# scverse/scanpy

Hardware: AMD Instinct MI355X
Metric: cells/sec through pca+neighbors+leiden, 1M x 2k CSR (higher is better)
Workload: dtype bf16x3

## Files before the change

### include/scanpy_amd.h

```cpp
#ifndef SCANPY_AMD_H
#define SCANPY_AMD_H

#include <stddef.h>
#include <stdint.h>

#ifdef __cplusplus
extern "C" {
#endif

typedef struct ihipStream_t* scamd_stream_t;

#define SCAMD_OK 0
#define SCAMD_EINVAL (-1)
#define SCAMD_EWORKSPACE (-2)
#define SCAMD_EHIP (-3)
#define SCAMD_EUNSUPPORTED (-4)
#define SCAMD_ECAPACITY (-5)
#define SCAMD_EINTERNAL (-6)

#define SCAMD_ABI_VERSION 1

int scamd_abi_version(void);
const char* scamd_last_error(void);
int scamd_device_count(void);

size_t scamd_knn_workspace_bytes(int64_t n, int d, int64_t n_query, int k);
int scamd_knn_l2_f32(const float* x, int64_t n, int d, int64_t ld_x,
                     int64_t q_begin, int64_t n_query, int k,
                     int32_t* out_idx, double* out_dist,
                     double cert_scale, int64_t* n_fallback_host,
                     void* workspace, size_t workspace_bytes, scamd_stream_t stream);
int scamd_knn_l2_ivf_f32(const float* x, int64_t n, int d, int64_t ld_x,
                         int64_t q_begin, int64_t n_query, int k, int nprobe,
                         int32_t* out_idx, double* out_dist, int64_t* n_fallback_host,
                         void* workspace, size_t workspace_bytes, scamd_stream_t stream);
float scamd_knn_last_select_ms(void);
double scamd_knn_last_select_pairs(void);
double scamd_knn_last_select_prepass_pairs(void);
int scamd_knn_last_select_engine(void);
int scamd_knn_last_second_tier_queries(void);
int scamd_knn_last_nprobe(void);
int scamd_knn_last_coarse(void);
void scamd_knn_cert_factors(int engine, double* cert_k, double* cert_k2, double* key_slack);
size_t scamd_knn_debug_b3_scores_workspace_bytes(int64_t n);
int scamd_knn_debug_b3_scores_f32(const float* x, int64_t n, int d, int64_t ld_x, int64_t q0, int nq, int64_t c0, int nc,
                                  float* out_scores, float* out_mu, float* out_cmax, void* workspace,
                                  size_t workspace_bytes, scamd_stream_t stream);
int scamd_knn_debug_cell_tables_sizes(int64_t n, int d, int64_t n_query, int k, int nprobe, int* n_cells, int64_t* n_img_max);
int scamd_knn_debug_cell_tables(int64_t n, int d, int64_t n_query, int k, int nprobe, const void* workspace,
                                size_t workspace_bytes, int32_t* out_labels, int32_t* out_row_cell, int32_t* out_cell_map,
                                float* out_cent, float* out_radius, int32_t* out_tile0, int32_t* out_ntiles, int32_t* out_order,
                                float* out_lb2, int32_t* out_perm, int64_t* n_img_rows_host, scamd_stream_t stream);
int scamd_knn_debug_sweep_tables(int64_t n, int d, int64_t n_query, int k, int nprobe, const void* workspace,
                                 size_t workspace_bytes, float* out_reach, int32_t* out_list_len, int32_t* out_sweep_order,
                                 float* out_sweep_lb2, scamd_stream_t stream);

size_t scamd_fuzzy_workspace_bytes(int64_t n, int k);
int scamd_fuzzy_simplicial_set_f32(const int32_t* knn_idx, const float* knn_dist, int64_t n, int k,
                                   int64_t* out_indptr, int32_t* out_indices, float* out_data,
                                   int64_t cap, float* out_sigma, float* out_rho, int64_t* nnz_host,
                                   void* workspace, size_t workspace_bytes, scamd_stream_t stream);
int scamd_fuzzy_weights_f32(const int32_t* knn_idx, const float* knn_dist, int64_t n_local, int k, int64_t row_begin,
                            int64_t n_total, const double* sum_all_dev, float* w, float* out_sigma, float* out_rho,
                            int32_t* out_count, scamd_stream_t stream);
size_t scamd_fuzzy_merge_workspace_bytes(int64_t n_local, int64_t cap);
int scamd_fuzzy_merge_rows_f32(const int32_t* knn_idx, const float* w, int64_t n_local, int k, const int64_t* in_indptr,
                               const int32_t* in_src, const float* in_w, int64_t* out_indptr, int32_t* out_indices,
                               float* out_data, int64_t cap, int64_t* nnz_host, void* workspace, size_t workspace_bytes,
                               scamd_stream_t stream);
int scamd_gauss_connectivities_f32(const int32_t* knn_idx, const float* knn_dist, int64_t n, int k, int64_t* out_indptr,
                                   int32_t* out_indices, float* out_data, int64_t cap, int64_t* nnz_host,
                                   void* workspace, size_t workspace_bytes, scamd_stream_t stream);
int scamd_jaccard_connectivities_f32(const int32_t* knn_idx, int64_t n, int k, int64_t* out_indptr,
                                     int32_t* out_indices, float* out_data, int64_t cap, int64_t* nnz_host,
                                     void* workspace, size_t workspace_bytes, scamd_stream_t stream);


int scamd_csr_row_stats_f32(const int64_t* indptr, const float* data, int64_t n_rows,
                            double* row_sum, double* row_sumsq, scamd_stream_t stream);
size_t scamd_csr_transpose_workspace_bytes(int64_t n, int64_t g, int64_t nnz);
int scamd_csr_transpose_f32(const int64_t* indptr, const int32_t* indices, const float* data,
                            int64_t n, int64_t g, int64_t nnz,
                            int64_t* t_indptr, int32_t* t_indices, float* t_data,
                            void* workspace, size_t workspace_bytes, scamd_stream_t stream);
int scamd_spmm_csr_f32(const int64_t* indptr, const int32_t* indices, const float* data,
// ... 246 lines not shown
```

### scanpy_amd/_lib.py

```python
from __future__ import annotations

import ctypes as C
from functools import lru_cache
from pathlib import Path

LIB_PATH = Path(__file__).resolve().parent / "_lib" / "libscanpy_amd.so"

_i64, _i32, _f64, _sz, _vp, _u64 = C.c_int64, C.c_int, C.c_double, C.c_size_t, C.c_void_p, C.c_uint64

SIGNATURES = {
    "scamd_abi_version": (_i32, []),
    "scamd_last_error": (C.c_char_p, []),
    "scamd_device_count": (_i32, []),
    "scamd_knn_workspace_bytes": (_sz, [_i64, _i32, _i64, _i32]),
    "scamd_knn_l2_f32": (_i32, [_vp, _i64, _i32, _i64, _i64, _i64, _i32, _vp, _vp, _f64, C.POINTER(_i64), _vp, _sz, _vp]),
    "scamd_knn_l2_ivf_f32": (_i32, [_vp, _i64, _i32, _i64, _i64, _i64, _i32, _i32, _vp, _vp, C.POINTER(_i64), _vp, _sz, _vp]),
    "scamd_knn_last_select_ms": (C.c_float, []),
    "scamd_knn_last_select_pairs": (_f64, []),
    "scamd_knn_last_select_prepass_pairs": (_f64, []),
    "scamd_knn_last_select_engine": (_i32, []),
    "scamd_knn_last_second_tier_queries": (_i32, []),
    "scamd_knn_last_nprobe": (_i32, []),
    "scamd_knn_last_coarse": (_i32, []),
    "scamd_knn_cert_factors": (None, [_i32, C.POINTER(_f64), C.POINTER(_f64), C.POINTER(_f64)]),
    "scamd_knn_debug_b3_scores_workspace_bytes": (_sz, [_i64]),
    "scamd_knn_debug_b3_scores_f32": (_i32, [_vp, _i64, _i32, _i64, _i64, _i32, _i64, _i32, _vp, _vp, _vp, _vp, _sz, _vp]),
    "scamd_knn_debug_cell_tables_sizes": (_i32, [_i64, _i32, _i64, _i32, _i32, C.POINTER(_i32), C.POINTER(_i64)]),
    "scamd_knn_debug_cell_tables": (_i32, [_i64, _i32, _i64, _i32, _i32, _vp, _sz, _vp, _vp, _vp, _vp, _vp, _vp, _vp, _vp, _vp, _vp,
                                           C.POINTER(_i64), _vp]),
    "scamd_knn_debug_sweep_tables": (_i32, [_i64, _i32, _i64, _i32, _i32, _vp, _sz, _vp, _vp, _vp, _vp, _vp]),
    "scamd_fuzzy_workspace_bytes": (_sz, [_i64, _i32]),
    "scamd_fuzzy_simplicial_set_f32": (_i32, [_vp, _vp, _i64, _i32, _vp, _vp, _vp, _i64, _vp, _vp, C.POINTER(_i64), _vp, _sz, _vp]),
    "scamd_fuzzy_weights_f32": (_i32, [_vp, _vp, _i64, _i32, _i64, _i64, _vp, _vp, _vp, _vp, _vp, _vp]),
    "scamd_fuzzy_merge_workspace_bytes": (_sz, [_i64, _i64]),
    "scamd_fuzzy_merge_rows_f32": (_i32, [_vp, _vp, _i64, _i32, _vp, _vp, _vp, _vp, _vp, _vp, _i64, C.POINTER(_i64), _vp, _sz, _vp]),
    "scamd_gauss_connectivities_f32": (_i32, [_vp, _vp, _i64, _i32, _vp, _vp, _vp, _i64, C.POINTER(_i64), _vp, _sz, _vp]),
    "scamd_jaccard_connectivities_f32": (_i32, [_vp, _i64, _i32, _vp, _vp, _vp, _i64, C.POINTER(_i64), _vp, _sz, _vp]),
    "scamd_csr_row_stats_f32": (_i32, [_vp, _vp, _i64, _vp, _vp, _vp]),
    "scamd_csr_transpose_workspace_bytes": (_sz, [_i64, _i64, _i64]),
    "scamd_csr_transpose_f32": (_i32, [_vp, _vp, _vp, _i64, _i64, _i64, _vp, _vp, _vp, _vp, _sz, _vp]),
    "scamd_spmm_csr_f32": (_i32, [_vp, _vp, _vp, _i64, _i64, _vp, _i32, _vp, _vp, _vp]),
    "scamd_spmm_f64acc_workspace_bytes": (_sz, [_i64, _i64, _i32]),
    "scamd_spmm_csr_f32_f64acc": (_i32, [_vp, _vp, _vp, _i64, _i64, _vp, _i32, _vp, _vp, _vp, _vp, _sz, _vp]),
    "scamd_csr_gram_workspace_bytes": (_sz, [_i64, _i64]),
    "scamd_csr_gram_f32": (_i32, [_vp, _vp, _vp, _i64, _i64, _i64, _i32, _vp, _i64, _vp, C.POINTER(C.c_float), _vp, _sz, _vp]),
    "scamd_eigh_topk_workspace_bytes": (_sz, [_i64, _i32]),
    "scamd_eigh_topk_f64": (_i32, [_vp, _i64, _i64, _i32, _u64, _f64, _vp, _vp, _vp, _vp, _sz, _vp]),
    "scamd_dense_debug_f64": (_i32, [_i32, _vp, _vp, _i32, _i32, _i32, _vp, _vp, C.POINTER(_i32), _vp]),
    "scamd_pca_csr_workspace_bytes": (_sz, [_i64, _i64, _i32]),
    "scamd_pca_csr_f32": (_i32, [_vp, _vp, _vp, _i64, _i64, _i64, _i32, _i32, _u64, _f64, _vp, _vp, _vp, _vp, _vp, _vp, _vp, _sz, _vp]),
    "scamd_pca_solve_gram_workspace_bytes": (_sz, [_i64, _i32]),
    "scamd_pca_solve_gram_f64": (_i32, [_vp, _i64, _vp, _i64, _i64, _i32, _i32, _i32, _u64, _f64, _vp, _vp, _vp, _vp, _vp, _vp, _vp, _vp, _vp, _sz, _vp]),
    "scamd_spectral_embedding_workspace_bytes": (_sz, [_i64, _i64, _i32]),
    "scamd_spectral_embedding_f32": (_i32, [_vp, _vp, _vp, _i64, _i64, _i32, _u64, _f64, _i32, _i32, _vp, C.POINTER(_f64), _vp, _sz, _vp]),
    "scamd_transitions_sym_workspace_bytes": (_sz, [_i64, _i64]),
    "scamd_transitions_sym_f32": (_i32, [_vp, _vp, _vp, _i64, _i64, _i32, _vp, _vp, _vp, _sz, _vp]),
    "scamd_diffmap_workspace_bytes": (_sz, [_i64, _i64, _i32]),
    "scamd_diffmap_f32": (_i32, [_vp, _vp, _vp, _i64, _i64, _i32, _u64, _f64, _i32, _i32, _vp, _vp, C.POINTER(_f64), _vp, _sz, _vp]),
    "scamd_dpt_pseudotime_workspace_bytes": (_sz, [_i64]),
    "scamd_dpt_pseudotime_f32": (_i32, [_vp, _vp, _i64, _i32, _i64, _i64, _vp, _i32, _vp, _vp, _sz, _vp]),
    "scamd_colsum_workspace_bytes": (_sz, [_i32]),
    "scamd_colsum_f32_f64": (_i32, [_vp, _i64, _i32, _vp, _vp, _sz, _vp]),
# ... 129 lines not shown
```

### scanpy_amd/csrc/knn.hip

```cpp
#include "common.h"

#include <algorithm>
#include <cmath>
#include <cstdlib>
#include <memory>
#include <type_traits>
#include <vector>

struct KnnLast {
  float select_ms = -1.f;
  double select_pairs = -1.0, select_prepass_pairs = -1.0;
  int select_engine = -1, second_tier = 0;
  int coarse = 0;
  int nprobe = 0;
};
static thread_local KnnLast g_last;

namespace scamd {

using f32x16 = __attribute__((ext_vector_type(16))) float;
using f32x4 = __attribute__((ext_vector_type(4))) float;
using i32x4 = __attribute__((ext_vector_type(4))) int;
typedef __attribute__((__vector_size__(8 * sizeof(__bf16)))) __bf16 bf16x8;

// ... 1915 lines not shown
    const int64_t i = i0 + (int64_t)t * 1024;
    if (cell[t] < 0) continue;
    const int c = cell[t];
    const int pos = row_off[c] + l_row[c] + rk[t];
    perm[pos] = (int)i;
    if (qk[t] >= 0) {
      qpos[slot_off[c] + l_slot[c] + qk[t]] = pos;
      if (qrow) qrow[i - q0] = pos;
    }
  }
}

__global__ void ivf_t2_count_kernel(const int* __restrict__ flag_list, int n_flag, int64_t q0, const int* __restrict__ labels,
                                    const int* __restrict__ cell_map, int* __restrict__ cnt, int* __restrict__ cell_out,
                                    int* __restrict__ pos_out) {
  const int j = blockIdx.x * blockDim.x + threadIdx.x;
  if (j >= n_flag) return;
  const int c = cell_map[labels[q0 + flag_list[j]]];
  cell_out[j] = c;
  pos_out[j] = atomicAdd(&cnt[c], 1);
}
__global__ void ivf_t2_fill_kernel(const int* __restrict__ flag_list, int n_flag, const int* __restrict__ cell_in,
                                   const int* __restrict__ pos_in, const int* __restrict__ slot_off,
                                   const int* __restrict__ qrow, int* __restrict__ qpos) {
  const int j = blockIdx.x * blockDim.x + threadIdx.x;
  if (j >= n_flag) return;
  qpos[slot_off[cell_in[j]] + pos_in[j]] = qrow[flag_list[j]];
}
__global__ void knn_iota_kernel(int* __restrict__ a, int n) {
  const int i = blockIdx.x * blockDim.x + threadIdx.x;
  if (i < n) a[i] = i;
}

__global__ void ivf_pack_image_kernel(const float* __restrict__ x, const float* __restrict__ mu, int d, int64_t ld,
                                      int H, int HP, int DPL,
                                      int64_t n_img, const int* __restrict__ perm, const int* __restrict__ labels,
                                      const int* __restrict__ cell_map, const float* __restrict__ cent,
                                      float* __restrict__ xp, unsigned int* __restrict__ cmax_bits,
                                      unsigned int* __restrict__ radius_bits, int b3) {
  const int lane = threadIdx.x & 63, sub = lane & 15;
  const int64_t grp = ((int64_t)blockIdx.x * blockDim.x + threadIdx.x) >> 4;
  const int64_t ngrp = ((int64_t)gridDim.x * blockDim.x) >> 4;
  float wmax = 0.f;
  const int64_t rpg = (n_img + ngrp - 1) / ngrp;
  const int64_t r_lo = grp * rpg, r_hi = r_lo + rpg < n_img ? r_lo + rpg : n_img;
  int run_cell = -1;
  unsigned int run_rb = 0u;
  auto flush_radius = [&]() {
    if (sub == 0 && run_cell >= 0 && run_rb > 0u) atomicMax(&radius_bits[run_cell], run_rb);
  };
  int src_next = r_lo < r_hi ? perm[r_lo] : -1;
  for (int64_t r = r_lo; r < r_hi; ++r) {
    const int src = src_next;
    src_next = r + 1 < r_hi ? perm[r + 1] : -1;
    double s = 0.0;
    float dc2 = 0.f;
    int cell = 0;
    if (src >= 0) {
      cell = cell_map[labels[src]];
      for (int c = sub; c < d; c += 16) {
        const float v = x[(int64_t)src * ld + c];
        const float vc = __fsub_rn(v, mu[c]);
        s += (double)vc * (double)vc;
        const float df = v - cent[cell * d + c];
        dc2 = fmaf(df, df, dc2);
      }
    }
#pragma unroll
    for (int o = 8; o > 0; o >>= 1) {
      s += __shfl_xor(s, o);
      dc2 += __shfl_xor(dc2, o);
    }
    const float nf = (src >= 0) ? (float)s : INFINITY;
    pack_image_row(xp, r, sub, 16, b3, H, HP, DPL, d, src < 0, nf,
                   [&](int dim) { return src >= 0 ? __fsub_rn(x[(int64_t)src * ld + dim], mu[dim]) : 0.f; });
    if (src >= 0) {
      wmax = fmaxf(wmax, nf);
      const unsigned int rb = __float_as_uint(sqrtf(dc2) * 1.0001f + 1e-6f);
      if (cell != run_cell) {
        flush_radius();
        run_cell = cell;
        run_rb = 0u;
      }
      run_rb = max(run_rb, rb);
    }
  }
  flush_radius();
#pragma unroll
  for (int o = 32; o > 0; o >>= 1) wmax = fmaxf(wmax, __shfl_xor(wmax, o));
  if (lane == 0 && wmax > 0.f && __float_as_uint(wmax) > __hip_atomic_load(cmax_bits, __ATOMIC_RELAXED, __HIP_MEMORY_SCOPE_AGENT))
    atomicMax(cmax_bits, __float_as_uint(wmax));
}


struct KnnPlan {
  int H, TC, NW, KP;
  bool reg;
  bool b3;
  bool thr_margin_env;
  int thr_rank;
  int row_dwords;
  int64_t n_pad, nq_pad;
  bool ivf;
  int nprobe;
  int n_cells;
  int64_t n_img_max, n_slot_max;
};

static bool knn_plan(int64_t n, int d, int64_t n_query, int k, KnnPlan* p, int nprobe = 0) {
  p->nprobe = 0;
  if (d <= 16) p->H = 8;
  else if (d <= 32) p->H = 16;
  else if (d <= 50) p->H = 25;
  else if (d <= 64) p->H = 32;
  else if (d <= 128) p->H = 64;
  else if (d <= 256) p->H = 128;
  else return false;
  p->TC = (p->H == 128) ? 32 : ((p->H == 64) ? 64 : 128);
  if (k <= 24) { p->KP = 32; p->NW = 8; }
  else if (k <= 56) { p->KP = 64; p->NW = 4; }
// ... 89 lines not shown
    b->block_perm = ws.take<int>(block_perm_capacity(p));
    b->qorder = ws.take<int>((size_t)p.n_slot_max);
    b->reach = ws.take<float>((size_t)p.n_cells * p.n_cells);
    b->list_len = ws.take<int>((size_t)p.n_cells);
    b->reach_chunks = ws.take<int>((size_t)p.n_cells);
    b->sweep_order = ws.take<int>((size_t)p.n_cells * p.n_cells);
    b->sweep_lb2 = ws.take<float>((size_t)p.n_cells * p.n_cells);
  }
  if (p.ivf && p.b3) {
    b->qrow = ws.take<int>((size_t)n_query);
    b->xp2 = ws.take<float>((size_t)p.n_img_max * RegCfg<25>::DPL);
    b->flag_list2 = ws.take<int>((size_t)n_query);
    b->t2_cell = ws.take<int>((size_t)n_query);
    b->t2_pos = ws.take<int>((size_t)n_query);
    b->t2_ints = ws.take<int>((size_t)p.n_cells * 2 + 8);
  }
}

struct CellTables {
  int *counts, *qcounts;
  int* cell_map;
  int *row_off, *row_cur;
  int *slot_off, *slot_cur;
  int *tile0, *ntiles;
  const float* radius;
  int *work, *first_block, *n_blocks;
};
static CellTables cell_tables(const KnnBuffers& b, size_t nc) {
  int* const ci = b.cell_ints;
  int* const ca = b.cell_aux;
  return {ci, ci + nc, ci + 2 * nc, ci + 3 * nc, ci + 4 * nc, ci + 5 * nc, ci + 6 * nc, ci + 7 * nc, reinterpret_cast<int*>(b.sums),
          reinterpret_cast<const float*>(b.radius_bits), ca, ca + nc, ca + 2 * nc};
}

template <int H, int TC, int NW, int KP>
static int launch_select(const KnnPlan& p, const KnnBuffers& b, int64_t q_begin, hipStream_t s) {
  using C = SelectCfg<H, TC, NW, KP>;
  auto kern = knn_select_kernel<H, TC, NW, KP>;
  SCAMD_HIP_CHECK(hipFuncSetAttribute(reinterpret_cast<const void*>(kern),
                                      hipFuncAttributeMaxDynamicSharedMemorySize, (int)C::LDS_BYTES));
  const int n_tiles = (int)(p.n_pad / TC);
  const int grid = (int)(p.nq_pad / C::QB);
  hipLaunchKernelGGL(kern, dim3(grid), dim3(C::NT), C::LDS_BYTES, s, b.xp, b.cn, n_tiles, p.n_pad,
                     q_begin, b.cand_idx, b.cand_tau);
  SCAMD_LAUNCH_CHECK();
  return SCAMD_OK;
}

template <int H, int TC>
static int dispatch_kp(const KnnPlan& p, const KnnBuffers& b, int64_t q_begin, hipStream_t s) {
  switch (p.KP) {
    case 32: return launch_select<H, TC, 8, 32>(p, b, q_begin, s);
    case 64: return launch_select<H, TC, 4, 64>(p, b, q_begin, s);
    case 128: return launch_select<H, TC, 2, 128>(p, b, q_begin, s);
    default: return launch_select<H, (TC < 64 ? TC : 64), 1, 288>(p, b, q_begin, s);
  }
}
template <>
int dispatch_kp<128, 32>(const KnnPlan& p, const KnnBuffers& b, int64_t q_begin, hipStream_t s) {
  if (p.KP == 128) return launch_select<128, 32, 2, 128>(p, b, q_begin, s);
  return launch_select<128, 32, 1, 288>(p, b, q_begin, s);
}

template <int H, int TC_, int WPS, bool B3 = false>
static int launch_select_reg_mode(const KnnPlan& p, const KnnBuffers& b, int64_t q_begin, hipStream_t s) {
  using C = RegCfg<H, TC_, B3>;
// ... 207 lines not shown
      hipLaunchKernelGGL(ivf_count_kernel, dim3((unsigned)ceil_div(c.n, 4096)), dim3(1024), 0, c.s, b.labels, c.n, nc, c.q_begin,
                         c.q_begin + c.n_query, t.counts, t.qcounts);
      SCAMD_LAUNCH_CHECK();
    }
    SCAMD_HIP_CHECK(hipMemcpyAsync(h_cnt->data(), t.counts, sizeof(int) * 2 * nc, hipMemcpyDeviceToHost, c.s));
    SCAMD_HIP_CHECK(hipMemcpyAsync(h_cent->data(), b.cent, sizeof(float) * nc * c.d, hipMemcpyDeviceToHost, c.s));
    SCAMD_HIP_CHECK(hipStreamSynchronize(c.s));
    return SCAMD_OK;
  }
  int upload_tables(const CellLayout& L) const {
    hipStream_t s = c.s;
    const size_t cell_bytes = sizeof(int) * nc;
    const std::pair<int*, const std::vector<int>*> per_cell[] = {
        {t.cell_map, &L.cell_map}, {t.row_off, &L.row_off}, {t.slot_off, &L.slot_off}, {t.tile0, &L.tile0}, {t.ntiles, &L.ntiles},
        {b.reach_chunks, &L.reach_chunks}};
    for (const auto& [dst, src] : per_cell) SCAMD_HIP_CHECK(hipMemcpyAsync(dst, src->data(), cell_bytes, hipMemcpyHostToDevice, s));
    SCAMD_HIP_CHECK(hipMemcpyAsync(b.block_cell, L.block_cell.data(), sizeof(int) * L.block_cell.size(), hipMemcpyHostToDevice, s));
    SCAMD_HIP_CHECK(hipMemcpyAsync(t.first_block, L.blocks.data(), 2 * cell_bytes, hipMemcpyHostToDevice, s));
    SCAMD_HIP_CHECK(hipMemsetAsync(t.row_cur, 0, cell_bytes, s));
    SCAMD_HIP_CHECK(hipMemsetAsync(t.slot_cur, 0, cell_bytes, s));
    SCAMD_HIP_CHECK(hipMemsetAsync(b.perm, 0xff, sizeof(int) * L.rows, s));
    SCAMD_HIP_CHECK(hipMemsetAsync(b.qpos, 0xff, sizeof(int) * L.slots, s));
    SCAMD_HIP_CHECK(hipMemsetAsync(b.radius_bits, 0, sizeof(unsigned int) * nc, s));
    SCAMD_HIP_CHECK(hipMemsetAsync(b.counters + KC_PAIRS, 0, sizeof(int) * (KC_LAUNCH_ORDER_ERR - KC_PAIRS), s));
    SCAMD_HIP_CHECK(hipStreamSynchronize(s));
    return SCAMD_OK;
  }
  int build_image_and_orders(const CellLayout& L) const {
    hipStream_t s = c.s;
    hipLaunchKernelGGL(ivf_scatter_kernel, dim3((unsigned)ceil_div(c.n, 1024 * SCATTER_ROWS)), dim3(1024), 0, s, b.labels, c.n, t.cell_map,
                       t.row_off, t.row_cur, c.q_begin, c.q_begin + c.n_query, t.slot_off, t.slot_cur, b.perm, b.qpos, b.qrow, nc);
    SCAMD_LAUNCH_CHECK();
    const int blocks = (int)std::min<int64_t>((L.rows + 15) / 16, 256 * 16);
    hipLaunchKernelGGL(ivf_pack_image_kernel, dim3(blocks), dim3(256), 0, s, c.x, b.mu, c.d, c.ld, p.H, (p.H + 1 + 3) / 4 * 4, p.row_dwords, L.rows, b.perm, b.labels,
                       t.cell_map, b.cent, b.xp, b.cmax, b.radius_bits, p.b3 ? 1 : 0);
    SCAMD_LAUNCH_CHECK();
    int npow = 1;
    while (npow < nc) npow <<= 1;
    const size_t olds = (size_t)npow * 8;
    SCAMD_HIP_CHECK(hipFuncSetAttribute(reinterpret_cast<const void*>(ivf_cell_order_kernel),
                                        hipFuncAttributeMaxDynamicSharedMemorySize, (int)olds));
    hipLaunchKernelGGL(ivf_cell_order_kernel, dim3(nc), dim3(256), olds, s, b.cent, c.d, t.radius, t.ntiles, nc, b.cell_order, b.cell_lb2,
                       t.work, p.nprobe);
    SCAMD_LAUNCH_CHECK();
    if (p.nprobe == 0) {
      hipLaunchKernelGGL(ivf_reach_init_kernel, dim3(nc), dim3(256), 0, s, t.radius, t.ntiles, nc, b.cell_order, b.cell_lb2, b.reach,
                         b.list_len);
      SCAMD_LAUNCH_CHECK();
      hipLaunchKernelGGL(reach, dim3(L.n_reach_blocks), dim3(256), 0, s, c.x, c.d, c.ld, b.cent, t.tile0, t.ntiles, nc, b.perm,
                         b.cell_order, b.list_len, b.reach_chunks, b.reach);
      SCAMD_LAUNCH_CHECK();
      SCAMD_HIP_CHECK(hipFuncSetAttribute(reinterpret_cast<const void*>(ivf_sweep_order_kernel),
                                          hipFuncAttributeMaxDynamicSharedMemorySize, (int)olds));
      hipLaunchKernelGGL(ivf_sweep_order_kernel, dim3(nc), dim3(256), olds, s, b.cent, c.d, t.radius, t.ntiles, nc, b.cell_order, b.cell_lb2,
                         b.reach, b.sweep_order, b.sweep_lb2, t.work);
      SCAMD_LAUNCH_CHECK();
    }
    hipLaunchKernelGGL(ivf_block_order_kernel, dim3(1), dim3(1024), 0, s, t.work, t.first_block, t.n_blocks, nc, b.block_perm, L.n_launch,
                       L.xcd_mode, b.counters + KC_LAUNCH_ORDER_ERR);
    SCAMD_LAUNCH_CHECK();
    return SCAMD_OK;
  }
  int choose_coarse(const CellLayout& L, bool* coarse) const {
    *coarse = p.b3 && env_is("SCAMD_KNN_COARSE", '1');
    if (!p.b3 || *coarse || env_is("SCAMD_KNN_COARSE", '0')) return SCAMD_OK;
    std::vector<int> h_work(nc);
    SCAMD_HIP_CHECK(hipMemcpyAsync(h_work.data(), t.work, sizeof(int) * nc, hipMemcpyDeviceToHost, c.s));
    SCAMD_HIP_CHECK(hipStreamSynchronize(c.s));
    double num = 0.0, den = 0.0;
// ... 117 lines not shown
static int run_ivf_tier2(const KnnPlan& p, const KnnBuffers& b, const KnnCall& c, int n_flag, int64_t rows, int* n_flag2_host) {
  using C = RegCfg<25, 64, false>;
  const int nc = p.n_cells;
  const CellTables t = cell_tables(b, nc);
  hipStream_t s = c.s;
  int* cnt2 = b.t2_ints;
  int* slot_off2 = b.t2_ints + nc;
  int* ctr2 = b.t2_ints + 2 * nc;
  *n_flag2_host = 0;
  SCAMD_HIP_CHECK(hipMemsetAsync(cnt2, 0, sizeof(int) * nc, s));
  SCAMD_HIP_CHECK(hipMemsetAsync(ctr2, 0, sizeof(int) * KC_HOST_SLOTS, s));
  hipLaunchKernelGGL(ivf_t2_count_kernel, dim3((unsigned)ceil_div(n_flag, 256)), dim3(256), 0, s, b.flag_list, n_flag, c.q_begin,
                     b.labels, t.cell_map, cnt2, b.t2_cell, b.t2_pos);
  SCAMD_LAUNCH_CHECK();
  t2_dbg(s, __LINE__);
  std::vector<int> h_cnt(nc), h_slot_off, h_block_cell;
  SCAMD_READBACK_NOW(h_cnt.data(), cnt2, sizeof(int) * nc, s);
  const int64_t slots = layout_query_blocks(h_cnt, &h_slot_off, &h_block_cell);
  const int n_blocks = (int)h_block_cell.size();
  if (n_blocks == 0) return SCAMD_OK;
  SCAMD_REQUIRE(slots <= p.n_slot_max, SCAMD_EWORKSPACE, "knn: second-tier query layout exceeds its bound");
  SCAMD_HIP_CHECK(hipMemcpyAsync(slot_off2, h_slot_off.data(), sizeof(int) * nc, hipMemcpyHostToDevice, s));
  SCAMD_HIP_CHECK(hipMemcpyAsync(b.block_cell, h_block_cell.data(), sizeof(int) * n_blocks, hipMemcpyHostToDevice, s));
  SCAMD_HIP_CHECK(hipMemsetAsync(b.qpos, 0xff, sizeof(int) * slots, s));
  SCAMD_HIP_CHECK(hipStreamSynchronize(s));
  hipLaunchKernelGGL(ivf_t2_fill_kernel, dim3((unsigned)ceil_div(n_flag, 256)), dim3(256), 0, s, b.flag_list, n_flag, b.t2_cell,
                     b.t2_pos, slot_off2, b.qrow, b.qpos);
  SCAMD_LAUNCH_CHECK();
  t2_dbg(s, __LINE__);
  hipLaunchKernelGGL(knn_iota_kernel, dim3((unsigned)ceil_div(n_blocks, 256)), dim3(256), 0, s, b.block_perm, n_blocks);
  SCAMD_LAUNCH_CHECK();
  t2_dbg(s, __LINE__);
  const int blocks = (int)std::min<int64_t>((rows + 3) / 4, 256 * 16);
  hipLaunchKernelGGL(ivf_pack_image_kernel, dim3(blocks), dim3(256), 0, s, c.x, b.mu, c.d, c.ld, 25, C::HP, C::DPL, rows, b.perm,
                     b.labels, t.cell_map, b.cent, b.xp2, b.cmax, b.radius_bits, 0);
  SCAMD_LAUNCH_CHECK();
  t2_dbg(s, __LINE__);
  auto kern = knn_select_reg_kernel<25, 64, 3, true, false>;
  const size_t lds = C::LDS_BYTES + 64 + IVF_META_BYTES;
  SCAMD_HIP_CHECK(hipFuncSetAttribute(reinterpret_cast<const void*>(kern), hipFuncAttributeMaxDynamicSharedMemorySize,
                                      (int)lds));
  IvfArgs iv = ivf_args(b, t, nc, c.d, p.nprobe);
  iv.pairs = reinterpret_cast<unsigned long long*>(ctr2 + KC_PAIRS);
  iv.prepass_tiles = 16;
  iv.prepass_min2 = 1;
  iv.n_slots = n_blocks;
  const int thr_rank = std::min(32, std::max(1, c.k + 6));
  hipLaunchKernelGGL(kern, dim3(n_blocks), dim3(C::NT), lds, s, b.xp2, (int)(rows / 64), rows, c.q_begin, thr_rank, b.cand_idx,
                     b.cand_tau, iv);
  SCAMD_LAUNCH_CHECK();
  t2_dbg(s, __LINE__);
  if (int rc = launch_rerank_rows(b, c, thr_rank, CERT_K_F32, 0.0, b.flag_list2, ctr2 + KC_UNCERTIFIED, b.flag_list, n_flag)) return rc;
  t2_dbg(s, __LINE__);
  SCAMD_READBACK_NOW(n_flag2_host, ctr2 + KC_UNCERTIFIED, sizeof(int), s);
  return SCAMD_OK;
}

static int stage_mean_and_image(const KnnPlan& p, const KnnBuffers& b, const KnnCall& c) {
  hipStream_t s = c.s;
  SCAMD_HIP_CHECK(hipMemsetAsync(b.cmax, 0, 16, s));
  SCAMD_HIP_CHECK(hipMemsetAsync(b.counters, 0, sizeof(int) * KC_HOST_SLOTS, s));
  hipLaunchKernelGGL(knn_colsum_kernel, dim3(MEAN_BLOCKS), dim3(1024), 0, s, c.x, c.n, c.d, c.ld, b.mean_partial);
  SCAMD_LAUNCH_CHECK();
  hipLaunchKernelGGL(knn_colmean_kernel, dim3(1), dim3(KNN_MAX_D), 0, s, b.mean_partial, c.n, c.d, b.mu);
  SCAMD_LAUNCH_CHECK();
  if (p.ivf) return SCAMD_OK;
  const int blocks = (int)std::min<int64_t>((p.n_pad + 3) / 4, 256 * 16);
  if (p.reg) {
    const int HP = (p.H + 1 + 3) / 4 * 4;
// ... 299 lines not shown
  SCAMD_HIP_CHECK(d2d(out_order, b.cell_order, cell_bytes * nc));
  SCAMD_HIP_CHECK(d2d(out_lb2, b.cell_lb2, cell_bytes * nc));
  if (rows > 0) SCAMD_HIP_CHECK(d2d(out_perm, b.perm, sizeof(int) * (size_t)rows));
  hipLaunchKernelGGL(scamd::knn_debug_row_cell_kernel, dim3((unsigned)ceil_div(n, 256)), dim3(256), 0, s, b.labels, t.cell_map, n, nc,
                     out_row_cell);
  SCAMD_LAUNCH_CHECK();
  return SCAMD_OK;
}

extern "C" int scamd_knn_debug_sweep_tables(int64_t n, int d, int64_t n_query, int k, int nprobe, const void* workspace,
                                            size_t workspace_bytes, float* out_reach, int32_t* out_list_len, int32_t* out_sweep_order,
                                            float* out_sweep_lb2, scamd_stream_t stream) {
  int nc = 0;
  int64_t n_img_max = 0;
  if (int rc = scamd_knn_debug_cell_tables_sizes(n, d, n_query, k, nprobe, &nc, &n_img_max)) return rc;
  SCAMD_REQUIRE(nprobe <= 0, SCAMD_EINVAL, "knn debug sweep tables: the approximate mode (nprobe=%d) builds none", nprobe);
  SCAMD_REQUIRE(workspace && out_reach && out_list_len && out_sweep_order && out_sweep_lb2, SCAMD_EINVAL,
                "knn debug sweep tables: null pointer");
  KnnPlan p;
  knn_plan(n, d, n_query, k, &p, 0);
  Workspace ws(const_cast<void*>(workspace), workspace_bytes);
  KnnBuffers b;
  knn_carve(ws, p, n_query, &b);
  SCAMD_REQUIRE(ws.ok, SCAMD_EWORKSPACE, "knn debug sweep tables: workspace %zu < required %zu", workspace_bytes, ws.used());
  hipStream_t s = stream;
  const size_t cell_bytes = sizeof(int) * (size_t)nc;
  SCAMD_HIP_CHECK(hipMemcpyAsync(out_reach, b.reach, cell_bytes * nc, hipMemcpyDeviceToDevice, s));
  SCAMD_HIP_CHECK(hipMemcpyAsync(out_list_len, b.list_len, cell_bytes, hipMemcpyDeviceToDevice, s));
  SCAMD_HIP_CHECK(hipMemcpyAsync(out_sweep_order, b.sweep_order, cell_bytes * nc, hipMemcpyDeviceToDevice, s));
  SCAMD_HIP_CHECK(hipMemcpyAsync(out_sweep_lb2, b.sweep_lb2, cell_bytes * nc, hipMemcpyDeviceToDevice, s));
  return SCAMD_OK;
}

namespace scamd {
__global__ void mfma_layout_kernel(int* mismatches) {
  const int lane = threadIdx.x & 63;
  const int i = lane & 31, kk = lane >> 5;
  float a = (float)(i + 100 * kk + 1);
  float bval = (float)(3 * i + 7 * kk + 2);
  f32x16 acc;
#pragma unroll
  for (int r = 0; r < 16; ++r) {
    int row = (r & 3) + 8 * (r >> 2) + 4 * kk;
    acc[r] = (float)(1000 * row + i);
  }
  acc = __builtin_amdgcn_mfma_f32_32x32x2f32(a, bval, acc, 0, 0, 0);
  int bad = 0;
#pragma unroll
  for (int r = 0; r < 16; ++r) {
    int row = (r & 3) + 8 * (r >> 2) + 4 * kk;
    int col = i;
    float expect = (float)(1000 * row + col);
    for (int k2 = 0; k2 < 2; ++k2) expect += (float)(row + 100 * k2 + 1) * (float)(3 * col + 7 * k2 + 2);
    if (acc[r] != expect) ++bad;
  }
  if (bad) atomicAdd(mismatches, bad);
}
}

extern "C" int scamd_selftest_mfma_layout(scamd_stream_t stream) {
  int* d_bad = nullptr;
  SCAMD_HIP_CHECK(hipMalloc(&d_bad, sizeof(int)));
  SCAMD_HIP_CHECK(hipMemsetAsync(d_bad, 0, sizeof(int), stream));
  hipLaunchKernelGGL(scamd::mfma_layout_kernel, dim3(1), dim3(64), 0, stream, d_bad);
  int h_bad = -1;
  hipError_t e = hipGetLastError();
// ... 14 lines not shown
```

Baseline: 24.64 million.

## Stage IVF image rows through LDS with batched async loads and tile-based cell lookup

Rewrites the IVF image packing kernel to fetch batches of four permuted rows into LDS with global_load_lds. It now derives each row's cell by binary-searching and walking the cell tile tables instead of gathering labels and cell_map per row. Centroids and the mean are cached in registers and LDS, and the centered values are reused from LDS when writing the packed row, instead of re-reading x. This adds a d<=64 limit, extra LDS and wave barriers, and a debug entry point for checking the packed image.

After: 24.78 million, median of 6. Within noise of the previous version (+0.6%).

```diff
diff --git a/include/scanpy_amd.h b/include/scanpy_amd.h
--- a/include/scanpy_amd.h
+++ b/include/scanpy_amd.h
@@ -51,6 +51,9 @@
                                 size_t workspace_bytes, int32_t* out_labels, int32_t* out_row_cell, int32_t* out_cell_map,
                                 float* out_cent, float* out_radius, int32_t* out_tile0, int32_t* out_ntiles, int32_t* out_order,
                                 float* out_lb2, int32_t* out_perm, int64_t* n_img_rows_host, scamd_stream_t stream);
+int scamd_knn_debug_image(int64_t n, int d, int64_t n_query, int k, int nprobe, const void* workspace, size_t workspace_bytes,
+                          int64_t n_img_rows, const float* x, int64_t ld_x, int repack_workgroups, float* out_norm_max,
+                          uint32_t* out_image, int* row_dwords_host, scamd_stream_t stream);
 int scamd_knn_debug_sweep_tables(int64_t n, int d, int64_t n_query, int k, int nprobe, const void* workspace,
                                  size_t workspace_bytes, float* out_reach, int32_t* out_list_len, int32_t* out_sweep_order,
                                  float* out_sweep_lb2, scamd_stream_t stream);
diff --git a/scanpy_amd/_lib.py b/scanpy_amd/_lib.py
--- a/scanpy_amd/_lib.py
+++ b/scanpy_amd/_lib.py
@@ -28,6 +28,7 @@
     "scamd_knn_debug_cell_tables_sizes": (_i32, [_i64, _i32, _i64, _i32, _i32, C.POINTER(_i32), C.POINTER(_i64)]),
     "scamd_knn_debug_cell_tables": (_i32, [_i64, _i32, _i64, _i32, _i32, _vp, _sz, _vp, _vp, _vp, _vp, _vp, _vp, _vp, _vp, _vp, _vp,
                                            C.POINTER(_i64), _vp]),
+    "scamd_knn_debug_image": (_i32, [_i64, _i32, _i64, _i32, _i32, _vp, _sz, _i64, _vp, _i64, _i32, _vp, _vp, C.POINTER(_i32), _vp]),
     "scamd_knn_debug_sweep_tables": (_i32, [_i64, _i32, _i64, _i32, _i32, _vp, _sz, _vp, _vp, _vp, _vp, _vp]),
     "scamd_fuzzy_workspace_bytes": (_sz, [_i64, _i32]),
     "scamd_fuzzy_simplicial_set_f32": (_i32, [_vp, _vp, _i64, _i32, _vp, _vp, _vp, _i64, _vp, _vp, C.POINTER(_i64), _vp, _sz, _vp]),
diff --git a/scanpy_amd/csrc/knn.hip b/scanpy_amd/csrc/knn.hip
--- a/scanpy_amd/csrc/knn.hip
+++ b/scanpy_amd/csrc/knn.hip
@@ -1971,60 +1971,124 @@
   if (i < n) a[i] = i;
 }
 
-__global__ void ivf_pack_image_kernel(const float* __restrict__ x, const float* __restrict__ mu, int d, int64_t ld,
-                                      int H, int HP, int DPL,
-                                      int64_t n_img, const int* __restrict__ perm, const int* __restrict__ labels,
-                                      const int* __restrict__ cell_map, const float* __restrict__ cent,
-                                      float* __restrict__ xp, unsigned int* __restrict__ cmax_bits,
-                                      unsigned int* __restrict__ radius_bits, int b3) {
-  const int lane = threadIdx.x & 63, sub = lane & 15;
+constexpr int PACK_BATCH = 4;
+constexpr int PACK_VPL = 4;
+constexpr int PACK_SRC = 0, PACK_CELL = 1;
+__global__ __launch_bounds__(256, 8) void ivf_pack_image_kernel(const float* __restrict__ x, const float* __restrict__ mu, int d, int64_t ld,
+                                                             int H, int HP, int DPL, int64_t n_img, const int* __restrict__ perm,
+                                                             const int* __restrict__ cell_tile0, const int* __restrict__ cell_ntiles,
+                                                             int n_cells, const float* __restrict__ cent, float* __restrict__ xp,
+                                                             unsigned int* __restrict__ cmax_bits,
+                                                             unsigned int* __restrict__ radius_bits, int b3) {
+  __shared__ float strips[4][PACK_BATCH][PACK_VPL][4][16];
+  __shared__ float metas[256 / 16][PACK_BATCH][2];
+  const int lane = threadIdx.x & 63, sub = lane & 15, grp4 = lane >> 4;
+  float(*strip)[PACK_VPL][4][16] = strips[__builtin_amdgcn_readfirstlane(threadIdx.x >> 6)];
+  float(*meta)[2] = metas[threadIdx.x >> 4];
+  __shared__ float mus[4][16 * PACK_VPL];
+  float* mu_w = mus[__builtin_amdgcn_readfirstlane(threadIdx.x >> 6)];
+  mu_w[lane] = mu[lane < d ? lane : d - 1];
   const int64_t grp = ((int64_t)blockIdx.x * blockDim.x + threadIdx.x) >> 4;
   const int64_t ngrp = ((int64_t)gridDim.x * blockDim.x) >> 4;
-  float wmax = 0.f;
-  const int64_t rpg = (n_img + ngrp - 1) / ngrp;
-  const int64_t r_lo = grp * rpg, r_hi = r_lo + rpg < n_img ? r_lo + rpg : n_img;
-  int run_cell = -1;
-  unsigned int run_rb = 0u;
+  const int rpg = (int)((n_img + ngrp - 1) / ngrp), r_last = (int)n_img - 1;
+  const int r_lo = (int)(grp * rpg < n_img ? grp * rpg : n_img);
+  const int r_hi = r_lo + rpg < (int)n_img ? r_lo + rpg : (int)n_img;
+  const int tile_lo = (r_lo < r_last ? r_lo : r_last) >> 6;
+  int clo = 0, chi = n_cells;
+  for (int w = n_cells; w > 1; w = (w + 15) / 16) {
+    const int step = (chi - clo + 15) / 16;
+    const int pc = clo + sub * step;
+    const bool le = pc < chi && cell_tile0[pc < n_cells ? pc : n_cells - 1] <= tile_lo;
+    int cnt = __popc((unsigned int)(__ballot(le) >> (lane & 48)) & 0xffffu);
+    cnt = cnt > 1 ? cnt : 1;
+    chi = chi < clo + cnt * step ? chi : clo + cnt * step;
+    clo += (cnt - 1) * step;
+  }
+  int cell = clo;
+  int cell_end = cell_tile0[cell] + cell_ntiles[cell];
+  __shared__ unsigned int runs[256 / 16][3];
+  unsigned int* run = runs[threadIdx.x >> 4];
+  if (sub == 0) {
+    run[0] = 0xffffffffu;
+    run[1] = 0u;
+    run[2] = 0u;
+  }
   auto flush_radius = [&]() {
-    if (sub == 0 && run_cell >= 0 && run_rb > 0u) atomicMax(&radius_bits[run_cell], run_rb);
+    if (sub == 0 && (int)run[0] >= 0 && run[1] > 0u) atomicMax(&radius_bits[(int)run[0]], run[1]);
   };
-  int src_next = r_lo < r_hi ? perm[r_lo] : -1;
-  for (int64_t r = r_lo; r < r_hi; ++r) {
-    const int src = src_next;
-    src_next = r + 1 < r_hi ? perm[r + 1] : -1;
-    double s = 0.0;
-    float dc2 = 0.f;
-    int cell = 0;
-    if (src >= 0) {
-      cell = cell_map[labels[src]];
-      for (int c = sub; c < d; c += 16) {
-        const float v = x[(int64_t)src * ld + c];
-        const float vc = __fsub_rn(v, mu[c]);
-        s += (double)vc * (double)vc;
-        const float df = v - cent[cell * d + c];
-        dc2 = fmaf(df, df, dc2);
-      }
-    }
-#pragma unroll
-    for (int o = 8; o > 0; o >>= 1) {
-      s += __shfl_xor(s, o);
-      dc2 += __shfl_xor(dc2, o);
-    }
-    const float nf = (src >= 0) ? (float)s : INFINITY;
-    pack_image_row(xp, r, sub, 16, b3, H, HP, DPL, d, src < 0, nf,
-                   [&](int dim) { return src >= 0 ? __fsub_rn(x[(int64_t)src * ld + dim], mu[dim]) : 0.f; });
-    if (src >= 0) {
-      wmax = fmaxf(wmax, nf);
-      const unsigned int rb = __float_as_uint(sqrtf(dc2) * 1.0001f + 1e-6f);
-      if (cell != run_cell) {
-        flush_radius();
-        run_cell = cell;
-        run_rb = 0u;
-      }
-      run_rb = max(run_rb, rb);
+  const auto cc = [&](int t) { return sub + 16 * t < d ? sub + 16 * t : d - 1; };
+  float cen[PACK_VPL] = {};
+  const auto perm_of = [&](int r0) { return perm[r0 + (sub & (PACK_BATCH - 1)) < r_last ? r0 + (sub & (PACK_BATCH - 1)) : r_last]; };
+  int src_next = perm_of(r_lo);
+  const int n_batch = (rpg + PACK_BATCH - 1) / PACK_BATCH;
+  for (int bi = 0; bi < n_batch; ++bi) {
+    const int r0 = r_lo + bi * PACK_BATCH;
+    __builtin_amdgcn_wave_barrier();
+    const int cell_before = cell;
+#pragma unroll
+    for (int j = 0; j < PACK_BATCH; ++j) {
+      const int r = r0 + j;
+      const int sj = __shfl(src_next, (lane & 48) + j);
+      const int src = r < r_hi ? sj : -1;
+      if (r < r_hi)
+        while ((r >> 6) >= cell_end && cell + 1 < n_cells) cell_end += cell_ntiles[++cell];
+      const float* xrow = x + (int64_t)(src >= 0 ? src : 0) * ld;
+#pragma unroll
+      for (int t = 0; t < PACK_VPL; ++t)
+        if (sub + 16 * t < d) __builtin_amdgcn_global_load_lds(xrow + sub + 16 * t, SCAMD_LDS_PTR(&strip[j][t][0][0]), 4, 0, 0);
+      if (sub == 0) {
+        meta[j][PACK_SRC] = __int_as_float(src);
+        meta[j][PACK_CELL] = __int_as_float(cell);
+      }
+    }
+    if (cell != cell_before || bi == 0) {
+#pragma unroll
+      for (int t = 0; t < PACK_VPL; ++t) cen[t] = cent[cell * d + cc(t)];
+    }
+    src_next = perm_of(r0 + PACK_BATCH);
+    __builtin_amdgcn_s_waitcnt(0);
+    __builtin_amdgcn_wave_barrier();
+#pragma unroll 1
+    for (int j = 0; j < PACK_BATCH; ++j) {
+      const int src = __float_as_int(meta[j][PACK_SRC]), row_cell = __float_as_int(meta[j][PACK_CELL]);
+      double s = 0.0;
+      float dc2 = 0.f;
+#pragma unroll
+      for (int t = 0; t < PACK_VPL; ++t) {
+        float vc = 0.f;
+        if (src >= 0 && sub + 16 * t < d) {
+          const float v = strip[j][t][grp4][sub];
+          vc = __fsub_rn(v, mu_w[sub + 16 * t]);
+          s += (double)vc * (double)vc;
+          const float df = v - (row_cell == cell ? cen[t] : cent[row_cell * d + cc(t)]);
+          dc2 = fmaf(df, df, dc2);
+        }
+        strip[j][t][grp4][sub] = vc;
+      }
+#pragma unroll
+      for (int o = 8; o > 0; o >>= 1) {
+        s += __shfl_xor(s, o);
+        dc2 += __shfl_xor(dc2, o);
+      }
+      __builtin_amdgcn_wave_barrier();
+      if (r0 + j >= r_hi) continue;
+      const float nf = (src >= 0) ? (float)s : INFINITY;
+      pack_image_row(xp, (int64_t)(r0 + j), sub, 16, b3, H, HP, DPL, d, src < 0, nf, [&](int dim) { return strip[j][dim >> 4][grp4][dim & 15]; });
+      if (src >= 0 && sub == 0) {
+        if (nf > __uint_as_float(run[2])) run[2] = __float_as_uint(nf);
+        const unsigned int rb = __float_as_uint(sqrtf(dc2) * 1.0001f + 1e-6f);
+        if (row_cell != (int)run[0]) {
+          flush_radius();
+          run[0] = (unsigned int)row_cell;
+          run[1] = 0u;
+        }
+        run[1] = max(run[1], rb);
+      }
     }
   }
   flush_radius();
+  __builtin_amdgcn_wave_barrier();
+  float wmax = __uint_as_float(run[2]);
 #pragma unroll
   for (int o = 32; o > 0; o >>= 1) wmax = fmaxf(wmax, __shfl_xor(wmax, o));
   if (lane == 0 && wmax > 0.f && __float_as_uint(wmax) > __hip_atomic_load(cmax_bits, __ATOMIC_RELAXED, __HIP_MEMORY_SCOPE_AGENT))
@@ -2180,6 +2244,14 @@
   return {ci, ci + nc, ci + 2 * nc, ci + 3 * nc, ci + 4 * nc, ci + 5 * nc, ci + 6 * nc, ci + 7 * nc, reinterpret_cast<int*>(b.sums),
           reinterpret_cast<const float*>(b.radius_bits), ca, ca + nc, ca + 2 * nc};
 }
+static int launch_pack_image(const KnnBuffers& b, const CellTables& t, int nc, const float* x, int d, int64_t ld, int H, int row_dwords,
+                             int64_t rows, float* xp, bool b3, int blocks, hipStream_t s) {
+  SCAMD_REQUIRE(d <= 16 * PACK_VPL && rows >= 64 && rows < (int64_t)1 << 30 && nc >= 1, SCAMD_EINTERNAL, "knn: image of %lld rows, d=%d, %d cells", (long long)rows, d, nc);
+  hipLaunchKernelGGL(ivf_pack_image_kernel, dim3(blocks), dim3(256), 0, s, x, b.mu, d, ld, H, (H + 1 + 3) / 4 * 4, row_dwords, rows, b.perm,
+                     t.tile0, t.ntiles, nc, b.cent, xp, b.cmax, b.radius_bits, b3 ? 1 : 0);
+  SCAMD_LAUNCH_CHECK();
+  return SCAMD_OK;
+}
 
 template <int H, int TC, int NW, int KP>
 static int launch_select(const KnnPlan& p, const KnnBuffers& b, int64_t q_begin, hipStream_t s) {
@@ -2453,9 +2525,7 @@
                        t.row_off, t.row_cur, c.q_begin, c.q_begin + c.n_query, t.slot_off, t.slot_cur, b.perm, b.qpos, b.qrow, nc);
     SCAMD_LAUNCH_CHECK();
     const int blocks = (int)std::min<int64_t>((L.rows + 15) / 16, 256 * 16);
-    hipLaunchKernelGGL(ivf_pack_image_kernel, dim3(blocks), dim3(256), 0, s, c.x, b.mu, c.d, c.ld, p.H, (p.H + 1 + 3) / 4 * 4, p.row_dwords, L.rows, b.perm, b.labels,
-                       t.cell_map, b.cent, b.xp, b.cmax, b.radius_bits, p.b3 ? 1 : 0);
-    SCAMD_LAUNCH_CHECK();
+    if (int rc = launch_pack_image(b, t, nc, c.x, c.d, c.ld, p.H, p.row_dwords, L.rows, b.xp, p.b3, blocks, s)) return rc;
     int npow = 1;
     while (npow < nc) npow <<= 1;
     const size_t olds = (size_t)npow * 8;
@@ -2639,9 +2709,7 @@
   SCAMD_LAUNCH_CHECK();
   t2_dbg(s, __LINE__);
   const int blocks = (int)std::min<int64_t>((rows + 3) / 4, 256 * 16);
-  hipLaunchKernelGGL(ivf_pack_image_kernel, dim3(blocks), dim3(256), 0, s, c.x, b.mu, c.d, c.ld, 25, C::HP, C::DPL, rows, b.perm,
-                     b.labels, t.cell_map, b.cent, b.xp2, b.cmax, b.radius_bits, 0);
-  SCAMD_LAUNCH_CHECK();
+  if (int rc = launch_pack_image(b, t, nc, c.x, c.d, c.ld, 25, C::DPL, rows, b.xp2, false, blocks, s)) return rc;
   t2_dbg(s, __LINE__);
   auto kern = knn_select_reg_kernel<25, 64, 3, true, false>;
   const size_t lds = C::LDS_BYTES + 64 + IVF_META_BYTES;
@@ -3007,6 +3075,46 @@
   return SCAMD_OK;
 }
 
+extern "C" int scamd_knn_debug_image(int64_t n, int d, int64_t n_query, int k, int nprobe, const void* workspace, size_t workspace_bytes,
+                                     int64_t n_img_rows, const float* x, int64_t ld_x, int repack_workgroups, float* out_norm_max,
+                                     uint32_t* out_image, int* row_dwords_host, scamd_stream_t stream) {
+  int nc = 0;
+  int64_t n_img_max = 0;
+  if (int rc = scamd_knn_debug_cell_tables_sizes(n, d, n_query, k, nprobe, &nc, &n_img_max)) return rc;
+  SCAMD_REQUIRE(workspace && out_norm_max && row_dwords_host && n_img_rows >= 0 && n_img_rows <= n_img_max, SCAMD_EINVAL,
+                "knn debug image: null pointer or %lld image rows beyond the plan's %lld", (long long)n_img_rows, (long long)n_img_max);
+  KnnPlan p;
+  knn_plan(n, d, n_query, k, &p, nprobe > 0 ? nprobe : 0);
+  Workspace ws(const_cast<void*>(workspace), workspace_bytes);
+  KnnBuffers b;
+  knn_carve(ws, p, n_query, &b);
+  SCAMD_REQUIRE(ws.ok, SCAMD_EWORKSPACE, "knn debug image: workspace %zu < required %zu", workspace_bytes, ws.used());
+  *row_dwords_host = p.row_dwords;
+  hipStream_t s = stream;
+  const CellTables t = cell_tables(b, (size_t)nc);
+  int last[2] = {0, 0};
+  {
+    const HostReadbackScope scope;
+    SCAMD_READBACK(&last[0], t.tile0 + nc - 1, sizeof(int), s);
+    SCAMD_READBACK(&last[1], t.ntiles + nc - 1, sizeof(int), s);
+    if (int rc = host_readback().sync(s)) return rc;
+  }
+  SCAMD_REQUIRE(n_img_rows == ((int64_t)last[0] + last[1]) * 64, SCAMD_EINVAL, "knn debug image: the image of this workspace has %lld rows, not %lld",
+                ((long long)last[0] + last[1]) * 64, (long long)n_img_rows);
+  if (repack_workgroups > 0) {
+    SCAMD_REQUIRE(x && ld_x >= d && repack_workgroups <= 65536, SCAMD_EINVAL, "knn debug image: repacking needs x, ld_x >= d and at most 65536 workgroups");
+    SCAMD_HIP_CHECK(hipMemsetAsync(b.cmax, 0, sizeof(unsigned int), s));
+    SCAMD_HIP_CHECK(hipMemsetAsync(b.radius_bits, 0, sizeof(unsigned int) * (size_t)nc, s));
+    SCAMD_HIP_CHECK(hipMemsetAsync(b.xp, 0xa5, sizeof(float) * (size_t)n_img_rows * p.row_dwords, s));
+    if (int rc = launch_pack_image(b, t, nc, x, d, ld_x, p.H, p.row_dwords, n_img_rows, b.xp, p.b3, repack_workgroups, s))
+      return rc;
+  }
+  SCAMD_HIP_CHECK(hipMemcpyAsync(out_norm_max, b.cmax, sizeof(float), hipMemcpyDeviceToDevice, s));
+  if (out_image && n_img_rows > 0)
+    SCAMD_HIP_CHECK(hipMemcpyAsync(out_image, b.xp, sizeof(float) * (size_t)n_img_rows * p.row_dwords, hipMemcpyDeviceToDevice, s));
+  return SCAMD_OK;
+}
+
 namespace scamd {
 __global__ void mfma_layout_kernel(int* mismatches) {
   const int lane = threadIdx.x & 63;
```
